# cvigilv/SimSpread.jl

Hardware: AMD Instinct MI355X
Metric: predicted edges/sec + achieved HBM GB/s, W*R SpMM (higher is better)
Workload: dtype f32

## Files before the change

simspread.jl_amd/csrc/kernels.hip:

```cpp
#include <type_traits>

#include "graph.hpp"

namespace ss {

static inline int grid_1d(int64_t work, int block, int cap = 256 * 16) {
  int64_t g = ceil_div(work, block);
  if (g < 1) g = 1;
  if (g > cap) g = cap;
  return (int)g;
}

#define SS_LAUNCH_CHECK()                                                             \
  do {                                                                                \
    hipError_t _e = hipGetLastError();                                                \
    if (_e != hipSuccess)                                                             \
      return fail(SS_EHIP, "%s:%d kernel launch: %s", __FILE__, __LINE__, hipGetErrorString(_e)); \
  } while (0)

template <class T>
__global__ void cutoff_kernel(const T* __restrict__ X, int64_t rows, int64_t cols, int64_t ld, T alpha,
                              int weighted, T* __restrict__ out, int64_t ldo) {
  const int64_t total = rows * cols;
  for (int64_t i = (int64_t)blockIdx.x * blockDim.x + threadIdx.x; i < total;
// ... 853 lines not shown
    const unsigned char* tb = tbl0 + par * W2_TBL;
    int fi, e, qoff;
    bool have = true;
    if (s < 16) {
      fi = 4 * s + (lane >> 4);
      e = lane & 15;
      qoff = 0;
    } else {
      const unsigned char* lst = lst0 + par * 128 + (s < 19 ? 0 : 64);
      const int pos = (s < 19 ? 16 * (s - 16) : 0) + (lane >> 2);
      fi = (int)lst[pos];
      have = fi != 255;
      fi = have ? fi : 0;
      e = lane & 3;
      qoff = s < 19 ? 16 : 20;
    }
    const unsigned* m = reinterpret_cast<const unsigned*>(tb + fi * 12);
    const int b = (int)m[0], n = (int)m[1];
    const float cf = __uint_as_float(m[2]);
    const int qe = qoff + e;
    const bool valid = have && 4 * qe < n;
    fetch(valid ? b + qe : lane, valid ? cf : 0.f, n - 4 * qe, oj, ov, ocf);
  };
  auto fold = [&](u2 j, f4 v, float cf) __attribute__((always_inline)) {
    atomicAdd(acc + (j.x & 0xffffu), (unsigned)cvt_rpi(cf * v.x));
    atomicAdd(acc + (j.x >> 16), (unsigned)cvt_rpi(cf * v.y));
    atomicAdd(acc + (j.y & 0xffffu), (unsigned)cvt_rpi(cf * v.z));
    atomicAdd(acc + (j.y >> 16), (unsigned)cvt_rpi(cf * v.w));
  };
  if (ngroups > 0) {
    raw_load(0, ra, rc);
    open_group(0);
#pragma unroll
    for (int i = 0; i < W2_D; ++i) gen(i, 0, sj[i], sv[i], sc[i]);
    for (int g = 0; g < ngroups; ++g) {
      const int par = g & 1;
#pragma unroll
      for (int s = 0; s < W2_STEPS; ++s) {
        if (s == W2_STEPS - W2_D) open_group(g + 1);
        fold(sj[s % W2_D], sv[s % W2_D], sc[s % W2_D]);
        if (s + W2_D < W2_STEPS) gen(s + W2_D, par, sj[s % W2_D], sv[s % W2_D], sc[s % W2_D]);
        else gen(s + W2_D - W2_STEPS, par ^ 1, sj[s % W2_D], sv[s % W2_D], sc[s % W2_D]);
      }
    }
  }
  float* orow = p.out + r * p.ld + j0;
  const int* iacc = reinterpret_cast<const int*>(acc);
  for (int j = lane; j < jn; j += 64) orow[j] = ((float)iacc[j] * unscale) * p.inv2[j0 + j];
}

template <class T>
static int transfer_block_waves(int64_t mrows, int SC, int* offs_bytes) {
  const int64_t ob = (((mrows + 1) * 4 + 15) / 16) * 16;
  const int64_t per_wave = (int64_t)(SC + 64) * (int64_t)sizeof(T);
  int64_t nw = ((int64_t)ctx().lds_per_block - ob) / per_wave;
  if (ob >= (int64_t)ctx().lds_per_block) nw = 0;
  if (nw > 16) nw = 16;
  if (const char* e = getenv("SS_TRANSFER_NW")) {
    const int v = atoi(e);
    if (v >= 1 && v < nw) nw = v;
  }
  *offs_bytes = (int)ob;
  return nw >= 8 ? (int)nw : 0;
}

template <class T>
int launch_transfer_block(const DevCsr<T>& L, const T* inv1, const DevChunked<T>& Mt, const T* inv2, int64_t row_begin,
                          int64_t nrows, int64_t nj, T* out, int64_t ld, T* coef, float xmax, bool fixed) {
  if (nrows <= 0 || nj <= 0) return SS_OK;
  int offs_bytes = 0;
  const int nw = transfer_block_waves<T>(Mt.rows, Mt.SC, &offs_bytes);
  if (nw == 0) return fail(SS_EUNSUPPORTED, "transfer_block: offsets + accumulators do not fit in LDS");
  TransferArgs<T> p{};
  p.nterms = 1;
  p.L[0] = view(L);
  p.M[0] = view(Mt);
  p.inv2 = inv2;
  p.row_begin = row_begin;
  p.nj = nj;
  p.SC = Mt.SC;
  p.nchunks = Mt.nchunks;
  p.out = out;
  p.ld = ld;
  const int64_t groups = ceil_div(nrows, (int64_t)nw);
  const int64_t grid = groups * p.nchunks;
  if (grid >= (1LL << 31)) return fail(SS_EUNSUPPORTED, "transfer grid too large; lower SS_TRANSFER_BYTES");
  path_add("transfer_block");
  hipLaunchKernelGGL(transfer_coef_kernel<T>, dim3(grid_1d(L.nnz > 0 ? L.nnz : 1, 256, 256 * 8)), dim3(256), 0, ctx().stream,
                     L.ptr.p, L.idx.p, L.val.p, inv1, row_begin, nrows, coef);
  SS_LAUNCH_CHECK();
  const size_t lds = (size_t)offs_bytes + (size_t)nw * (size_t)(p.SC + 64) * sizeof(T);
  constexpr bool CANFIX = std::is_same<T, float>::value;
  const bool fx = CANFIX && fixed;
  if (fx) path_add("fixed_point");
  if constexpr (std::is_same<T, float>::value) {
    auto envi = [](const char* k) { const char* e = getenv(k); return e ? atoi(e) : 0; };
    const int wide2 = envi("SS_TRANSFER_WIDE2"), wide = envi("SS_TRANSFER_WIDE"), qflat = envi("SS_TRANSFER_QFLAT");
    if ((wide2 > 0 || wide > 0 || qflat > 0) && fixed && Mt.align == 32 && Mt.len_ok) {
      const int64_t lens_bytes = ((Mt.rows * 2 + 15) / 16) * 16;
      const int64_t accb = ((((int64_t)p.SC + 4) * 4 + 15) / 16) * 16;
      const int64_t per_wave = wide2 > 0 ? accb + 2 * W2_TBL + 4 * 64
                               : wide > 0 ? accb + WIDE_META + WIDE_LIST : (int64_t)(p.SC + 64) * 4;
      const int64_t fixed_bytes = (int64_t)offs_bytes + lens_bytes + (wide > 0 && wide2 == 0 ? 64 : 0);
      int64_t nwf = ((int64_t)ctx().lds_per_block - fixed_bytes) / per_wave;
      if (nwf > 16) nwf = 16;
      if (const int v = envi("SS_TRANSFER_NW"); v >= 1 && v < nwf) nwf = v;
      if (nwf >= 8) {
        const int64_t fgrid = ceil_div(nrows, nwf) * p.nchunks;
        const size_t flds = (size_t)fixed_bytes + (size_t)nwf * (size_t)per_wave;
        const unsigned short* glen = Mt.len.p;
#define SS_TX_LAUNCH(KERNEL)                                                                                          \
  do {                                                                                                                \
    static std::atomic<bool> attr_done{false};                                                                        \
    if (!attr_done) {                                                                                                 \
      SS_HIP(hipFuncSetAttribute(reinterpret_cast<const void*>(&KERNEL), hipFuncAttributeMaxDynamicSharedMemorySize,  \
                                 160 * 1024));                                                                        \
      attr_done = true;                                                                                               \
    }                                                                                                                 \
    hipLaunchKernelGGL(KERNEL, dim3((unsigned)fgrid), dim3(64 * (int)nwf), flds, ctx().stream, p, (const float*)coef,  \
                       nrows, Mt.align, offs_bytes, (int)lens_bytes, xmax, glen);                                     \
  } while (0)
        if (wide2 > 0) {
          path_add("wide2");
          if (Mt.binary) SS_TX_LAUNCH((transfer_wide2_kernel<true>)); else SS_TX_LAUNCH((transfer_wide2_kernel<false>));
        } else if (wide > 0) {
          path_add("wide");
          if (wide == 2) { if (Mt.binary) SS_TX_LAUNCH((transfer_wide_kernel<2, true>)); else SS_TX_LAUNCH((transfer_wide_kernel<2, false>)); }
          else { if (Mt.binary) SS_TX_LAUNCH((transfer_wide_kernel<4, true>)); else SS_TX_LAUNCH((transfer_wide_kernel<4, false>)); }
        } else {
          path_add("qflat");
          if (Mt.binary) SS_TX_LAUNCH((transfer_qflat_kernel<float, 4, true>)); else SS_TX_LAUNCH((transfer_qflat_kernel<float, 4, false>));
        }
#undef SS_TX_LAUNCH
        SS_LAUNCH_CHECK();
        return SS_OK;
      }
    }
  }
  const int pu = transfer_u() == 4 ? 4 : 8;
#define SS_TB_LAUNCH(U, BINM, FIX)                                                                                    \
  do {                                                                                                                \
    static std::atomic<bool> attr_done{false};                                                                        \
    if (!attr_done) {                                                                                                 \
      SS_HIP(hipFuncSetAttribute(reinterpret_cast<const void*>(&transfer_block_kernel<T, U, BINM, FIX>),              \
                                 hipFuncAttributeMaxDynamicSharedMemorySize, 160 * 1024));                            \
      attr_done = true;                                                                                               \
    }                                                                                                                 \
    hipLaunchKernelGGL((transfer_block_kernel<T, U, BINM, FIX>), dim3((unsigned)grid), dim3(64 * nw), lds,            \
                       ctx().stream, p, (const T*)coef, nrows, Mt.align, offs_bytes, xmax);                           \
  } while (0)
#define SS_TB_BIN(U, FIX) do { if (Mt.binary) SS_TB_LAUNCH(U, true, FIX); else SS_TB_LAUNCH(U, false, FIX); } while (0)
#define SS_TB_FIX(U) do { if (fx) SS_TB_BIN(U, CANFIX); else SS_TB_BIN(U, false); } while (0)
  if (pu == 4) SS_TB_FIX(4);
  else SS_TB_FIX(8);
#undef SS_TB_FIX
#undef SS_TB_BIN
#undef SS_TB_LAUNCH
  SS_LAUNCH_CHECK();
  return SS_OK;
}

template <class T>
bool transfer_block_fits(int64_t mrows, int SC) {
  int ob = 0;
  return transfer_block_waves<T>(mrows, SC, &ob) > 0;
}

template <class T, bool LOO>
static int launch_transfer_variant(const TransferArgs<T>& p, unsigned grid, size_t lds, bool binm, bool dual) {
#define SS_TRANSFER_LAUNCH(U, BINM, DUAL)                                                               \
  hipLaunchKernelGGL((transfer_kernel<T, LOO, U, BINM, DUAL>), dim3(grid), dim3(TRANSFER_THREADS), lds, \
                     ctx().stream, p)
#define SS_TRANSFER_U(U)                                                                      \
  do {                                                                                        \
    if (binm) { if (dual) SS_TRANSFER_LAUNCH(U, true, true); else SS_TRANSFER_LAUNCH(U, true, false); } \
    else { if (dual) SS_TRANSFER_LAUNCH(U, false, true); else SS_TRANSFER_LAUNCH(U, false, false); }    \
  } while (0)
  if constexpr (std::is_same<T, float>::value && !LOO) {
    const char* eb = getenv("SS_TRANSFER_LD");
    if (eb && atoi(eb) == 1 && !dual) {
      path_add("buffer_loads");
      const bool fx = getenv("SS_TRANSFER_FIX1") && atoi(getenv("SS_TRANSFER_FIX1")) == 1 && p.nterms == 1 && !p.accumulate;
      if (fx) path_add("fixed_point");
#define SS_TL(U, BINM, FX) hipLaunchKernelGGL((transfer_kernel<T, LOO, U, BINM, false, FX, true>), dim3(grid), dim3(TRANSFER_THREADS), lds, ctx().stream, p)
      if (transfer_u(p.small_weighted != 0 && !LOO) == 4) {
        if (binm) { if (fx) SS_TL(4, true, true); else SS_TL(4, true, false); }
        else { if (fx) SS_TL(4, false, true); else SS_TL(4, false, false); }
      } else {
        if (binm) { if (fx) SS_TL(8, true, true); else SS_TL(8, true, false); }
        else { if (fx) SS_TL(8, false, true); else SS_TL(8, false, false); }
      }
#undef SS_TL
      SS_LAUNCH_CHECK();
      return SS_OK;
    }
    const char* e = getenv("SS_TRANSFER_FIX1");
    if (e && atoi(e) == 1 && p.nterms == 1 && !dual && !p.accumulate) {
      path_add("fixed_point");
      if (transfer_u(p.small_weighted != 0 && !LOO) == 4) {
        if (binm) hipLaunchKernelGGL((transfer_kernel<T, LOO, 4, true, false, true>), dim3(grid), dim3(TRANSFER_THREADS), lds, ctx().stream, p);
        else hipLaunchKernelGGL((transfer_kernel<T, LOO, 4, false, false, true>), dim3(grid), dim3(TRANSFER_THREADS), lds, ctx().stream, p);
      } else {
        if (binm) hipLaunchKernelGGL((transfer_kernel<T, LOO, 8, true, false, true>), dim3(grid), dim3(TRANSFER_THREADS), lds, ctx().stream, p);
        else hipLaunchKernelGGL((transfer_kernel<T, LOO, 8, false, false, true>), dim3(grid), dim3(TRANSFER_THREADS), lds, ctx().stream, p);
      }
      SS_LAUNCH_CHECK();
      return SS_OK;
    }
  }
  switch (transfer_u(p.small_weighted != 0 && !LOO)) {
    case 4: SS_TRANSFER_U(4); break;
    case 16: SS_TRANSFER_U(16); break;
    default: SS_TRANSFER_U(8); break;
  }
#undef SS_TRANSFER_U
#undef SS_TRANSFER_LAUNCH
  SS_LAUNCH_CHECK();
  return SS_OK;
}

template <class T>
int launch_transfer(int nterms, const DevCsr<T>* L[2], const T* inv1[2], const DevChunked<T>* Mt[2],
                    const T* inv2, int64_t row_begin, int64_t nrows, int64_t nj, T* out, int64_t ld,
                    const int* row_ids, bool accumulate) {
  if (nrows <= 0 || nj <= 0) return SS_OK;
  TransferArgs<T> p{};
  p.nterms = nterms;
  for (int t = 0; t < nterms; ++t) {
    p.L[t] = view(*L[t]);
    p.M[t] = view(*Mt[t]);
    p.inv1[t] = inv1[t];
    if (Mt[t]->SC != Mt[0]->SC || Mt[t]->nchunks != Mt[0]->nchunks)
      return fail(SS_EINVAL, "transfer operands were cut with different chunk sizes");
  }
  p.inv2 = inv2;
  p.row_begin = row_begin;
  p.row_ids = row_ids;
  p.nj = nj;
  p.SC = Mt[0]->SC;
  p.nchunks = Mt[0]->nchunks;
  p.out = out;
  p.ld = ld;
  p.accumulate = accumulate ? 1 : 0;
  p.xmax = 1.0f;
  {
    int64_t bytes = 0;
    bool weighted = false;
    for (int t = 0; t < nterms; ++t) {
      bytes += Mt[t]->stored * (int64_t)(2 + sizeof(T));
      weighted = weighted || !Mt[t]->binary;
    }
    p.small_weighted = (weighted && bytes <= (32LL << 20)) ? 1 : 0;
  }
  p.chunk_interleave = (getenv("SS_TRANSFER_ORDER") && atoi(getenv("SS_TRANSFER_ORDER")) == 0) ? 1 : 0;
  const int64_t grid = nrows * p.nchunks;
  if (grid >= (1LL << 31)) return fail(SS_EUNSUPPORTED, "transfer grid too large; lower SS_TRANSFER_BYTES");
  bool binm = true;
  for (int t = 0; t < nterms; ++t) binm = binm && Mt[t]->binary;
  const bool dual = transfer_dual();
  path_add("transfer");
  const size_t lds = (size_t)(p.SC + 64) * sizeof(T) * (dual ? 2 : 1);
  SS_TRY((launch_transfer_variant<T, false>(p, (unsigned)grid, lds, binm, dual)));
  return SS_OK;
}

template <class T>
int launch_transfer_loo(const DevCsr<T>& X, const DevChunked<T>& XT, const int* kf, const int* ks,
                        int64_t i_begin, int64_t nrows, T* out, int64_t ld) {
  if (nrows <= 0) return SS_OK;
  TransferArgs<T> p{};
  p.nterms = 1;
  p.L[0] = view(X);
  p.M[0] = view(XT);
  p.kf = kf;
  p.ks = ks;
  p.row_begin = i_begin;
  p.nj = X.rows;
  p.SC = XT.SC;
  p.nchunks = XT.nchunks;
  p.out = out;
  p.ld = ld;
  p.chunk_interleave = (getenv("SS_TRANSFER_ORDER") && atoi(getenv("SS_TRANSFER_ORDER")) == 0) ? 1 : 0;
  const int64_t grid = nrows * p.nchunks;
  if (grid >= (1LL << 31)) return fail(SS_EUNSUPPORTED, "transfer grid too large; lower SS_TRANSFER_BYTES");
  const bool dual = transfer_dual();
  path_add("transfer_loo");
  const size_t lds = (size_t)(p.SC + 64) * sizeof(T) * (dual ? 2 : 1) + (size_t)((p.SC + 31) / 32) * 4;
  SS_TRY((launch_transfer_variant<T, true>(p, (unsigned)grid, lds, XT.binary, dual)));
  return SS_OK;
}

template <class T, int QT>
struct alignas(sizeof(T) * QT) Vec {
  T v[QT];
};

template <class T>
struct SellArgs {
  const int* off;
  const unsigned short* idx;
  const T* val;
  int nslices, nchunks, KC;
  int64_t K, M, B;
  const T* R;
  int64_t ldr;
  T* F;
  int64_t ldf;
  const int* clean_deg;
  const int* out_rows;
};

constexpr int SELL_THREADS = 1024;
constexpr int SELL_NB = 4;
constexpr int SELL_QT_F32_DEFAULT = 4;
constexpr int SELL_ZERO_ROWS = 16;
constexpr int SELL_STAGE_IT = 5;

template <int H>
__device__ __forceinline__ unsigned half_shl(unsigned x, unsigned sh) {
  unsigned r;
  if (H == 0)
    asm("v_lshlrev_b32_sdwa %0, %1, %2 dst_sel:DWORD dst_unused:UNUSED_PAD src0_sel:DWORD src1_sel:WORD_0"
        : "=v"(r) : "v"(sh), "v"(x));
  else
    asm("v_lshlrev_b32_sdwa %0, %1, %2 dst_sel:DWORD dst_unused:UNUSED_PAD src0_sel:DWORD src1_sel:WORD_1"
        : "=v"(r) : "v"(sh), "v"(x));
  return r;
}

template <class T, int QT, bool BIN>
__global__ void __launch_bounds__(SELL_THREADS) spmm_sell_kernel(SellArgs<T> a) {
  constexpr int RB = (int)sizeof(T) * QT, NP = RB / 16;
  constexpr int STAGE_IT = NP == 2 ? 2 : SELL_STAGE_IT;
  constexpr int NBQ = NP == 2 ? 2 : SELL_NB;
  constexpr unsigned TSH = NP == 2 ? 5 : 4;
  static_assert(RB == 16 || (RB == 32 && sizeof(T) == 4), "tile row must be 16 bytes, or 32 bytes of fp32");
  extern __shared__ __align__(16) unsigned char smem_raw[];
  using V = Vec<T, QT>;
  V* tile = reinterpret_cast<V*>(smem_raw);
  const int tid = threadIdx.x, lane = tid & 63, wave = tid >> 6, nwaves = blockDim.x >> 6;
  const int64_t b0 = (int64_t)blockIdx.x * QT;
  const unsigned pid = NP == 2 ? (unsigned)(lane & 1) : 0u;

  for (int c = 0; c < a.nchunks; ++c) {
    const int64_t k0 = (int64_t)c * a.KC;
    const int kn = (int)((a.K - k0 < a.KC) ? (a.K - k0) : a.KC);
    if (c) __syncthreads();
    for (int kb = 0; kb < a.KC + SELL_ZERO_ROWS; kb += STAGE_IT * SELL_THREADS) {
      T stg[STAGE_IT][QT];
      const int klast = kn > 0 ? kn - 1 : 0;
#pragma unroll
      for (int it = 0; it < STAGE_IT; ++it) {
        const int k = kb + tid + it * SELL_THREADS;
        const int kk = k < kn ? k : klast;
#pragma unroll
        for (int q = 0; q < QT; ++q) {
          const int64_t b = (b0 + q < a.B) ? b0 + q : a.B - 1;
          stg[it][q] = kn > 0 ? a.R[b * a.ldr + k0 + kk] : T(0);
        }
      }
#pragma unroll
      for (int it = 0; it < STAGE_IT; ++it) {
        const int k = kb + tid + it * SELL_THREADS;
        if (k < a.KC + SELL_ZERO_ROWS) {
          V v;
#pragma unroll
          for (int q = 0; q < QT; ++q) v.v[q] = (k < kn && b0 + q < a.B) ? stg[it][q] : T(0);
          tile[k] = v;
        }
      }
    }
    __syncthreads();

    const int* off = a.off + (int64_t)c * a.nslices;
    const bool last = (c == a.nchunks - 1);
    for (int s = wave + nwaves * (int)blockIdx.y; s < a.nslices; s += nwaves * (int)gridDim.y) {
      const int o = __builtin_amdgcn_readfirstlane(off[s]);
      const int oe = __builtin_amdgcn_readfirstlane(off[s + 1]);
      T acc[QT];
#pragma unroll
      for (int q = 0; q < QT; ++q) acc[q] = T(0);
      const int64_t m = (int64_t)s * 64 + lane;
      T fprev[QT];
#pragma unroll
      for (int q = 0; q < QT; ++q) {
        fprev[q] = T(0);
        if (NP == 1 && c && m < a.M && b0 + q < a.B)
          fprev[q] = a.F[(a.out_rows ? (int64_t)a.out_rows[b0 + q] : b0 + q) * a.ldf + m];
      }
      const ushort4* ip = reinterpret_cast<const ushort4*>(a.idx) + (int64_t)o * 64 + lane;
      const Vec<T, 4>* vp = reinterpret_cast<const Vec<T, 4>*>(a.val) + (int64_t)o * 64 + lane;
      const uint2* ipw = reinterpret_cast<const uint2*>(ip);
      const int nq = oe - o;
      uint2 ia[NBQ], ib[NBQ];
      Vec<T, 4> wa[NBQ], wb[NBQ];
      auto fetch = [&](uint2 (&iq)[NBQ], Vec<T, 4> (&wq)[NBQ], int base) __attribute__((always_inline)) {
#pragma unroll
        for (int j = 0; j < NBQ; ++j) {
          iq[j] = ipw[(int64_t)(base + j) * 64];
          if (!BIN) wq[j] = vp[(int64_t)(base + j) * 64];
        }
      };
      auto gather = [&](const uint2 (&iq)[NBQ], const Vec<T, 4> (&wq)[NBQ], int cnt) __attribute__((always_inline)) {
        constexpr int PV = 16 / (int)sizeof(T);
        typedef T NV __attribute__((ext_vector_type(PV)));
        using LV = const __attribute__((address_space(3))) NV*;
        const unsigned lb = pid << 4;
        auto row = [&](unsigned addr) __attribute__((always_inline)) {
          V r;
          if (NP == 1) {
            const NV n = *(LV)(uintptr_t)addr;
#pragma unroll
            for (int q = 0; q < PV; ++q) r.v[q] = n[q];
          } else {
            const unsigned a0 = addr | lb;
            const NV n0 = *(LV)(uintptr_t)a0;
            const NV n1 = *(LV)(uintptr_t)(a0 ^ 16u);
#pragma unroll
            for (int q = 0; q < PV; ++q) { r.v[q] = n0[q]; r.v[PV + q] = n1[q]; }
          }
          return r;
        };
#pragma unroll
        for (int j = 0; j < NBQ; ++j) {
          if (j >= cnt) break;
          const V t0 = row(half_shl<0>(iq[j].x, TSH));
          const V t1 = row(half_shl<1>(iq[j].x, TSH));
          const V t2 = row(half_shl<0>(iq[j].y, TSH));
          const V t3 = row(half_shl<1>(iq[j].y, TSH));
          if (BIN) {
#pragma unroll
            for (int q = 0; q < QT; ++q) acc[q] += (t0.v[q] + t1.v[q]) + (t2.v[q] + t3.v[q]);
          } else {
#pragma unroll
            for (int q = 0; q < QT; ++q) {
              acc[q] = fma(wq[j].v[0], t0.v[q], acc[q]);
              acc[q] = fma(wq[j].v[1], t1.v[q], acc[q]);
              acc[q] = fma(wq[j].v[2], t2.v[q], acc[q]);
              acc[q] = fma(wq[j].v[3], t3.v[q], acc[q]);
            }
          }
          if (NP == 2) __builtin_amdgcn_sched_barrier(0);
        }
      };
      fetch(ia, wa, 0);
      fetch(ib, wb, NBQ);
      int u = 0;
      for (; u + 2 * NBQ <= nq; u += 2 * NBQ) {
        gather(ia, wa, NBQ);
        fetch(ia, wa, u + 2 * NBQ);
        gather(ib, wb, NBQ);
        fetch(ib, wb, u + 3 * NBQ);
      }
      {
        const int rest = nq - u;
        if (rest > 0) gather(ia, wa, rest < NBQ ? rest : NBQ);
        if (rest > NBQ) gather(ib, wb, rest - NBQ);
      }
      if (m < a.M) {
        const bool flag = last && a.clean_deg != nullptr && a.clean_deg[m] == 0;
#pragma unroll
        for (int q = 0; q < QT; ++q) {
          if (b0 + q < a.B) {
            T* f = a.F + (a.out_rows ? (int64_t)a.out_rows[b0 + q] : b0 + q) * a.ldf + m;
            const T mine = NP == 2 ? (pid ? acc[q ^ (QT / 2)] : acc[q]) : acc[q];
            const T r = mine + ((NP == 2 && c) ? *f : fprev[q]);
            *f = flag ? T(-99) : r;
          }
        }
      }
    }
  }
}

template <> int sell_tile_width<float>() {
  if (const char* e = getenv("SS_SELL_QT")) {
    const int v = atoi(e);
    if (v == 4 || v == 8) return v;
  }
  return SELL_QT_F32_DEFAULT;
}
template <> int sell_tile_width<double>() { return 2; }

template <class T>
int sell_max_chunk(int qt) {
  int64_t kc = (int64_t)(160 * 1024) / ((int64_t)qt * (int64_t)sizeof(T)) - SELL_ZERO_ROWS;
  if (kc > 65535 - (SELL_ZERO_ROWS - 1)) kc = 65535 - (SELL_ZERO_ROWS - 1);
  return (int)kc;
}

template <class T>
int launch_spmm_sell(const DevSell<T>& W, const T* R, int64_t ldr, int64_t B, T* F, int64_t ldf,
                     const int* clean_deg, const int* out_rows) {
  if (B <= 0 || W.rows <= 0) return SS_OK;
  path_add(W.sorted ? "spmm_sell_sorted" : "spmm_sell");
  const int QT = W.qt > 0 ? W.qt : (sizeof(T) == 4 ? 4 : 2);
  SellArgs<T> a{};
  a.off = W.off.p;
  a.idx = W.idx.p;
  a.val = W.val.p;
  a.nslices = W.nslices;
  a.nchunks = W.nchunks;
  a.KC = W.KC;
  a.K = W.cols;
  a.M = W.sorted ? W.vrows : W.rows;
  a.B = B;
  a.R = R;
  a.ldr = ldr;
  a.F = F;
  a.ldf = ldf;
  a.clean_deg = clean_deg;
  a.out_rows = out_rows;
  const size_t lds = (size_t)(W.KC + SELL_ZERO_ROWS) * QT * sizeof(T);
  if (lds > (size_t)160 * 1024) return fail(SS_EINVAL, "SELL chunk does not fit the LDS tile of %d columns", QT);
  const unsigned gx = (unsigned)ceil_div(B, QT);
  unsigned gy = 1;
  if ((int)gx < 2 * ctx().num_cu) {
    gy = (unsigned)ceil_div(2 * ctx().num_cu, (int64_t)gx);
    const unsigned maxy = (unsigned)ceil_div(W.nslices, SELL_THREADS / 64);
    if (gy > maxy) gy = maxy > 0 ? maxy : 1;
  }
  const dim3 grid(gx, gy);
  auto prepare = [](const void* fn) -> int {
    hipFuncAttributes fa{};
    SS_HIP(hipFuncGetAttributes(&fa, fn));
    if (fa.sharedSizeBytes != 0)
      return fail(SS_EUNSUPPORTED, "spmm_sell_kernel was built with %zu bytes of static LDS: its tile-relative LDS "
                  "addresses need the dynamic segment at LDS address 0", (size_t)fa.sharedSizeBytes);
    SS_HIP(hipFuncSetAttribute(fn, hipFuncAttributeMaxDynamicSharedMemorySize, 160 * 1024));
    return SS_OK;
  };
#define SS_SELL_LAUNCH(QTV, BINV, SLOT)                                                                      \
  do {                                                                                                       \
    static std::atomic<bool> attr_done{false};                                                               \
    if (!attr_done) {                                                                                        \
      SS_TRY(prepare(reinterpret_cast<const void*>(&spmm_sell_kernel<T, QTV, BINV>)));                       \
      attr_done = true;                                                                                      \
    }                                                                                                        \
    hipLaunchKernelGGL((spmm_sell_kernel<T, QTV, BINV>), grid, dim3(SELL_THREADS), lds, ctx().stream, a);    \
  } while (0)
  if constexpr (sizeof(T) == 4) {
    if (QT == 8) { if (W.binary) SS_SELL_LAUNCH(8, true, 0); else SS_SELL_LAUNCH(8, false, 1); }
    else if (QT == 4) { if (W.binary) SS_SELL_LAUNCH(4, true, 2); else SS_SELL_LAUNCH(4, false, 3); }
    else return fail(SS_EINVAL, "SELL tile width must be 4 or 8 (fp32)");
  } else {
    if (QT != 2) return fail(SS_EINVAL, "SELL tile width must be 2 (fp64)");
    if (W.binary) SS_SELL_LAUNCH(2, true, 0); else SS_SELL_LAUNCH(2, false, 1);
  }
#undef SS_SELL_LAUNCH
  SS_LAUNCH_CHECK();
  return SS_OK;
}

template <class T>
struct NarrowArgs {
  const int* off;
  const unsigned short* idx;
  const T* val;
  int64_t M, K;
  int KC, nchunks, B;
  const T* R;
  int64_t ldr;
  T* F;
  int64_t ldf;
  T* P;
};

constexpr int NARROW_THREADS = 1024;

template <int CTRL, int ROW_MASK = 0xF>
__device__ __forceinline__ float dpp_add(float v) {
  return v + __int_as_float(__builtin_amdgcn_update_dpp(0, __float_as_int(v), CTRL, ROW_MASK, 0xF, false));
}
template <int CTRL, int ROW_MASK = 0xF>
__device__ __forceinline__ double dpp_add(double v) {
  const long long b = __double_as_longlong(v);
  const int lo = __builtin_amdgcn_update_dpp(0, (int)(b & 0xffffffffll), CTRL, ROW_MASK, 0xF, false);
  const int hi = __builtin_amdgcn_update_dpp(0, (int)(b >> 32), CTRL, ROW_MASK, 0xF, false);
  return v + __longlong_as_double(((long long)hi << 32) | (unsigned int)lo);
}
template <int GL, class T>
__device__ __forceinline__ T lane_group_sum(T v) {
  static_assert(GL == 8 || GL == 16 || GL == 32 || GL == 64, "group of 8, 16, 32 or 64 lanes");
  v = dpp_add<0xB1>(v);
  v = dpp_add<0x4E>(v);
  v = dpp_add<0x141>(v);
  if constexpr (GL >= 16) v = dpp_add<0x140>(v);
  if constexpr (GL >= 32) v = dpp_add<0x142, 0xA>(v);
  if constexpr (GL >= 64) v = dpp_add<0x143, 0xC>(v);
  return v;
}

template <class T, int VEC, int GL, int UR, int NBQ>
__global__ void __launch_bounds__(NARROW_THREADS) spmm_chunked_narrow_kernel(NarrowArgs<T> a) {
  constexpr int BV = VEC;
  extern __shared__ __align__(16) unsigned char smem_raw[];
  T* tile = reinterpret_cast<T*>(smem_raw);
  using V = Vec<T, VEC>;
  const int tid = threadIdx.x, lane = tid & 63, wave = tid >> 6, nwaves = blockDim.x >> 6;
  const int c = blockIdx.x % a.nchunks;
  const int slot = blockIdx.x / a.nchunks, nslots = gridDim.x / a.nchunks;
  const int64_t k0 = (int64_t)c * a.KC;
  const int kn = (int)((a.K - k0 < a.KC) ? (a.K - k0) : a.KC);

  constexpr bool SWZ = (BV * sizeof(T) == 32);
  constexpr int HB = 16 / (int)sizeof(T);
  constexpr int PW16 = 16 / (int)sizeof(T);
  const bool packed = a.ldr == BV && a.B == BV &&
                      ((reinterpret_cast<uintptr_t>(a.R + k0 * a.ldr) & 15) == 0) && ((a.KC * BV) % PW16 == 0);
  if (packed) {
    using P16 = Vec<T, PW16>;
    const P16* __restrict__ src = reinterpret_cast<const P16*>(a.R + k0 * a.ldr);
    P16* dst = reinterpret_cast<P16*>(tile);
    const int npieces = ((a.KC + 1) * BV + PW16 - 1) / PW16, nfull = (kn * BV) / PW16;
    for (int i = tid; i < npieces; i += blockDim.x) {
      P16 v;
      if (i < nfull) {
        v = src[i];
      } else {
#pragma unroll
        for (int e = 0; e < PW16; ++e) {
          const int x = i * PW16 + e;
          v.v[e] = (x < kn * BV) ? a.R[k0 * a.ldr + x] : T(0);
        }
      }
      if ((i + 1) * PW16 <= (a.KC + 1) * BV) {
        dst[SWZ ? (i ^ ((i >> 4) & 1)) : i] = v;
      } else {
#pragma unroll
        for (int e = 0; e < PW16; ++e)
          if (i * PW16 + e < (a.KC + 1) * BV) tile[i * PW16 + e] = v.v[e];
      }
    }
  } else {
    for (int e = tid; e < (a.KC + 1) * BV; e += blockDim.x) {
      const int k = e / BV, b = e - k * BV;
      const T v = (k < kn && b < a.B) ? a.R[(k0 + k) * a.ldr + b] : T(0);
      if constexpr (SWZ) tile[k * BV + ((((b / HB) ^ (k >> 3)) & 1) * HB) + (b % HB)] = v;
      else tile[e] = v;
    }
  }
  __syncthreads();
  auto tile_row = [&](int k) __attribute__((always_inline)) {
    V r;
    if constexpr (SWZ) {
      using H = Vec<T, HB>;
      const int s = (k >> 3) & 1;
      const H lo = *reinterpret_cast<const H*>(&tile[k * BV + s * HB]);
      const H hi = *reinterpret_cast<const H*>(&tile[k * BV + (s ^ 1) * HB]);
#pragma unroll
      for (int i = 0; i < HB; ++i) { r.v[i] = lo.v[i]; r.v[HB + i] = hi.v[i]; }
    } else {
      r = *reinterpret_cast<const V*>(&tile[k * BV]);
    }
    return r;
  };

  const int* __restrict__ off = a.off + (int64_t)c * a.M;
  {
    constexpr int RPS = 64 / GL;
    const int sub = lane / GL, gl = lane % GL;
    const ushort4* __restrict__ ip = reinterpret_cast<const ushort4*>(a.idx);
    const Vec<T, 4>* __restrict__ vp = reinterpret_cast<const Vec<T, 4>*>(a.val);
    const int64_t stride = (int64_t)nslots * nwaves * RPS * UR;
    struct Bounds { int lo[UR], hi[UR]; };
    struct Quads { ushort4 iv[UR][NBQ]; Vec<T, 4> w[UR][NBQ]; unsigned mask; };
    auto bounds = [&](int64_t mb, Bounds& b) __attribute__((always_inline)) {
#pragma unroll
      for (int u = 0; u < UR; ++u) {
        const int64_t m = mb + u * RPS + sub;
        const int64_t mm = m < a.M ? m : a.M - 1;
        b.lo[u] = off[mm];
        b.hi[u] = off[mm + 1];
      }
    };
    auto issue = [&](int64_t mb, const Bounds& b, Quads& x) __attribute__((always_inline)) {
      unsigned mask = 0;
#pragma unroll
      for (int u = 0; u < UR; ++u) {
        const int oe = (mb + u * RPS + sub < a.M) ? b.hi[u] : b.lo[u];
#pragma unroll
        for (int nb = 0; nb < NBQ; ++nb) {
          const int q = b.lo[u] + gl + nb * GL;
          const bool in = q < oe;
          const int qq = in ? q : b.lo[u];
          {
            typedef unsigned nt_u2 __attribute__((ext_vector_type(2)));
            typedef T nt_t4 __attribute__((ext_vector_type(4)));
            const nt_u2 ii = __builtin_nontemporal_load(reinterpret_cast<const nt_u2*>(&ip[qq]));
            const nt_t4 ww = __builtin_nontemporal_load(reinterpret_cast<const nt_t4*>(&vp[qq]));
            x.iv[u][nb] = ushort4((unsigned short)(ii.x & 0xffffu), (unsigned short)(ii.x >> 16), (unsigned short)(ii.y & 0xffffu),
                                  (unsigned short)(ii.y >> 16));
            x.w[u][nb].v[0] = ww.x; x.w[u][nb].v[1] = ww.y; x.w[u][nb].v[2] = ww.z; x.w[u][nb].v[3] = ww.w;
          }
          mask |= in ? (1u << (u * NBQ + nb)) : 0u;
        }
        mask |= (b.lo[u] + NBQ * GL < oe) ? 0x80000000u : 0u;
      }
      x.mask = mask;
    };
    auto quad = [&](T (&acc)[VEC], const ushort4 jv, const Vec<T, 4> x) __attribute__((always_inline)) {
      const V r0 = tile_row((int)jv.x);
      const V r1 = tile_row((int)jv.y);
      const V r2 = tile_row((int)jv.z);
      const V r3 = tile_row((int)jv.w);
#pragma unroll
      for (int i = 0; i < VEC; ++i) {
        acc[i] = fma(x.v[0], r0.v[i], acc[i]);
        acc[i] = fma(x.v[1], r1.v[i], acc[i]);
        acc[i] = fma(x.v[2], r2.v[i], acc[i]);
        acc[i] = fma(x.v[3], r3.v[i], acc[i]);
      }
    };
    int64_t mb = ((int64_t)slot * nwaves + wave) * RPS * UR;
    Bounds bn;
    Quads xa, xb;
    if (mb < a.M) {
      Bounds b0;
      bounds(mb, b0);
      bounds(mb + stride < a.M ? mb + stride : mb, bn);
      issue(mb, b0, xa);
    }
    auto step = [&](const int64_t mb, const Quads& xc, Quads& xn) __attribute__((always_inline)) {
      const int64_t mb1 = mb + stride < a.M ? mb + stride : mb;
      const int64_t mb2 = mb + 2 * stride < a.M ? mb + 2 * stride : mb;
      Bounds bnn;
      bounds(mb2, bnn);
      issue(mb1, bn, xn);
      __builtin_amdgcn_sched_barrier(0);
      T acc[UR][VEC];
#pragma unroll
      for (int u = 0; u < UR; ++u) {
#pragma unroll
        for (int i = 0; i < VEC; ++i) acc[u][i] = T(0);
#pragma unroll
        for (int nb = 0; nb < NBQ; ++nb) {
          const bool has = (xc.mask >> (u * NBQ + nb)) & 1u;
          Vec<T, 4> w = xc.w[u][nb];
#pragma unroll
          for (int e = 0; e < 4; ++e) w.v[e] = has ? w.v[e] : T(0);
          quad(acc[u], xc.iv[u][nb], w);
        }
      }
      if (__any((int)(xc.mask >> 31))) {
#pragma unroll
        for (int u = 0; u < UR; ++u) {
          const int64_t m = mb + u * RPS + sub;
          if (m < a.M) {
            const int lo = off[m], hi = off[m + 1];
            for (int q = lo + gl + NBQ * GL; q < hi; q += GL) quad(acc[u], ip[q], vp[q]);
          }
        }
      }
#pragma unroll
      for (int u = 0; u < UR; ++u) {
#pragma unroll
        for (int i = 0; i < VEC; ++i) acc[u][i] = lane_group_sum<GL>(acc[u][i]);
        const int64_t m = mb + u * RPS + sub;
        if (gl == GL - 1 && m < a.M) {
          if (a.P) {
            T* p = a.P + ((int64_t)c * a.M + m) * BV;
#pragma unroll
            for (int i = 0; i < VEC; ++i) p[i] = acc[u][i];
          } else {
#pragma unroll
            for (int i = 0; i < VEC; ++i)
              if (i < a.B) a.F[m * a.ldf + i] = acc[u][i];
          }
        }
      }
      bn = bnn;
    };
    while (mb < a.M) {
      step(mb, xa, xb);
      mb += stride;
      if (mb >= a.M) break;
      step(mb, xb, xa);
      mb += stride;
    }
  }
}

template <class T, int BV>
__global__ void narrow_reduce_kernel(const T* __restrict__ P, int nchunks, int64_t M, int B, T* __restrict__ F,
                                     int64_t ldf) {
  using PV = Vec<T, BV>;
  for (int64_t m = (int64_t)blockIdx.x * blockDim.x + threadIdx.x; m < M; m += (int64_t)gridDim.x * blockDim.x) {
    PV s = *reinterpret_cast<const PV*>(P + m * BV);
    for (int c = 1; c < nchunks; ++c) {
      const PV t = *reinterpret_cast<const PV*>(P + ((int64_t)c * M + m) * BV);
#pragma unroll
      for (int e = 0; e < BV; ++e) s.v[e] += t.v[e];
    }
#pragma unroll
    for (int e = 0; e < BV; ++e)
      if (e < B) F[m * ldf + e] = s.v[e];
  }
}

template <class T>
int narrow_chunk_cols(int bv) {
  int64_t kc = (int64_t)(160 * 1024) / ((int64_t)bv * (int64_t)sizeof(T)) - 1;
  if (kc > 65535) kc = 65535;
  kc &= ~3LL;
  return (int)kc;
}

template <class T, int VEC, int GL, int UR, int NBQ = 1>
static int launch_narrow_variant(const NarrowArgs<T>& a, unsigned grid, size_t lds) {
  static std::atomic<bool> attr_set{false};
  if (!attr_set) {
    SS_HIP(hipFuncSetAttribute(reinterpret_cast<const void*>(&spmm_chunked_narrow_kernel<T, VEC, GL, UR, NBQ>),
                               hipFuncAttributeMaxDynamicSharedMemorySize, 160 * 1024));
    attr_set = true;
  }
  hipLaunchKernelGGL((spmm_chunked_narrow_kernel<T, VEC, GL, UR, NBQ>), dim3(grid), dim3(NARROW_THREADS), lds,
                     ctx().stream, a);
  SS_LAUNCH_CHECK();
  return SS_OK;
}

constexpr int narrow_ur(int elem, int vec, int nbq) {
  const int per_quad = 2 + elem;
  int ur = 4;
  while (ur > 1 && 2 * ur * nbq * per_quad + (ur + 4) * vec * (elem / 4) + 4 * ur + 24 > 124) ur >>= 1;
  return ur;
}

template <class T, int VEC>
static int launch_narrow_width(const NarrowArgs<T>& a, unsigned grid, size_t lds, double mean_quads) {
  constexpr int E = (int)sizeof(T);
  const double need = 1.1 * mean_quads + 1.0;
  if (need > 64.0) return launch_narrow_variant<T, VEC, 64, narrow_ur(E, VEC, 2), 2>(a, grid, lds);
  if (need > 32.0) return launch_narrow_variant<T, VEC, 64, narrow_ur(E, VEC, 1)>(a, grid, lds);
  if (need > 16.0) return launch_narrow_variant<T, VEC, 32, narrow_ur(E, VEC, 1)>(a, grid, lds);
  if (need > 8.0) return launch_narrow_variant<T, VEC, 16, narrow_ur(E, VEC, 1)>(a, grid, lds);
  return launch_narrow_variant<T, VEC, 8, narrow_ur(E, VEC, 1)>(a, grid, lds);
}

template <class T>
int launch_spmm_chunked_narrow(const DevChunked<T>& W, int bv, const T* R, int64_t ldr, int B, T* F, int64_t ldf,
                               DevBuf<T>& partial) {
  if (W.rows <= 0 || B <= 0) return SS_OK;
  if (W.align != 4) return fail(SS_EINVAL, "narrow operand must be quad-aligned");
  path_add("spmm_chunked_narrow");
  NarrowArgs<T> a{};
  a.off = W.off.p; a.idx = W.idx.p; a.val = W.val.p;
  a.M = W.rows; a.K = W.cols; a.KC = W.SC; a.nchunks = W.nchunks; a.B = B;
  a.R = R; a.ldr = ldr; a.F = F; a.ldf = ldf; a.P = nullptr;
  if (W.nchunks > 1) {
// ... 440 lines not shown
```

Baseline: 48.95 billion.

## Make SELL SpMM persistent and prefetch next tile's R staging during compute

The SELL SpMM kernel becomes persistent when gy==1: the grid is capped at the CU count and each workgroup loops over column tiles and chunks. Global loads of R for the first two staging rounds of the next tile or chunk are issued into registers before the following sync, so they overlap the current compute. This targets the exposed latency of filling the LDS tile and the cost of launching many short workgroups. In exchange it raises register pressure and launches fewer workgroups. It also adds env knobs, including a NOSTAGE debug variant.

```diff
diff --git a/simspread.jl_amd/csrc/kernels.hip b/simspread.jl_amd/csrc/kernels.hip
--- a/simspread.jl_amd/csrc/kernels.hip
+++ b/simspread.jl_amd/csrc/kernels.hip
@@ -1179,6 +1179,7 @@
   const T* val;
   int nslices, nchunks, KC;
   int64_t K, M, B;
+  int64_t ntiles;
   const T* R;
   int64_t ldr;
   T* F;
@@ -1205,10 +1206,11 @@
   return r;
 }
 
-template <class T, int QT, bool BIN>
+template <class T, int QT, bool BIN, bool NOSTAGE = false>
 __global__ void __launch_bounds__(SELL_THREADS) spmm_sell_kernel(SellArgs<T> a) {
   constexpr int RB = (int)sizeof(T) * QT, NP = RB / 16;
   constexpr int STAGE_IT = NP == 2 ? 2 : SELL_STAGE_IT;
+  constexpr int RND = STAGE_IT * SELL_THREADS;
   constexpr int NBQ = NP == 2 ? 2 : SELL_NB;
   constexpr unsigned TSH = NP == 2 ? 5 : 4;
   static_assert(RB == 16 || (RB == 32 && sizeof(T) == 4), "tile row must be 16 bytes, or 32 bytes of fp32");
@@ -1216,36 +1218,53 @@
   using V = Vec<T, QT>;
   V* tile = reinterpret_cast<V*>(smem_raw);
   const int tid = threadIdx.x, lane = tid & 63, wave = tid >> 6, nwaves = blockDim.x >> 6;
-  const int64_t b0 = (int64_t)blockIdx.x * QT;
   const unsigned pid = NP == 2 ? (unsigned)(lane & 1) : 0u;
 
-  for (int c = 0; c < a.nchunks; ++c) {
+  const int trows = a.KC + SELL_ZERO_ROWS;
+  auto request = [&](T (&stg)[STAGE_IT][QT], int64_t b0, int c, int kb) __attribute__((always_inline)) {
     const int64_t k0 = (int64_t)c * a.KC;
     const int kn = (int)((a.K - k0 < a.KC) ? (a.K - k0) : a.KC);
-    if (c) __syncthreads();
-    for (int kb = 0; kb < a.KC + SELL_ZERO_ROWS; kb += STAGE_IT * SELL_THREADS) {
-      T stg[STAGE_IT][QT];
-      const int klast = kn > 0 ? kn - 1 : 0;
-#pragma unroll
-      for (int it = 0; it < STAGE_IT; ++it) {
-        const int k = kb + tid + it * SELL_THREADS;
-        const int kk = k < kn ? k : klast;
-#pragma unroll
-        for (int q = 0; q < QT; ++q) {
-          const int64_t b = (b0 + q < a.B) ? b0 + q : a.B - 1;
-          stg[it][q] = kn > 0 ? a.R[b * a.ldr + k0 + kk] : T(0);
-        }
-      }
-#pragma unroll
-      for (int it = 0; it < STAGE_IT; ++it) {
-        const int k = kb + tid + it * SELL_THREADS;
-        if (k < a.KC + SELL_ZERO_ROWS) {
-          V v;
-#pragma unroll
-          for (int q = 0; q < QT; ++q) v.v[q] = (k < kn && b0 + q < a.B) ? stg[it][q] : T(0);
-          tile[k] = v;
-        }
-      }
+    const int klast = kn > 0 ? kn - 1 : 0;
+    const T* rq[QT];
+#pragma unroll
+    for (int q = 0; q < QT; ++q) rq[q] = a.R + ((b0 + q < a.B) ? b0 + q : a.B - 1) * a.ldr + k0;
+#pragma unroll
+    for (int it = 0; it < STAGE_IT; ++it) {
+      const int k = kb + tid + it * SELL_THREADS;
+      const unsigned kk = (unsigned)(k < kn ? k : klast);
+#pragma unroll
+      for (int q = 0; q < QT; ++q) stg[it][q] = NOSTAGE ? T(1) : rq[q][kk];
+    }
+  };
+  auto deposit = [&](const T (&stg)[STAGE_IT][QT], int64_t b0, int kn, int kb) __attribute__((always_inline)) {
+#pragma unroll
+    for (int it = 0; it < STAGE_IT; ++it) {
+      const int k = kb + tid + it * SELL_THREADS;
+      if (k < trows) {
+        V v;
+#pragma unroll
+        for (int q = 0; q < QT; ++q) v.v[q] = (k < kn && b0 + q < a.B) ? stg[it][q] : T(0);
+        tile[k] = v;
+      }
+    }
+  };
+
+  int64_t t = blockIdx.x;
+  if (t >= a.ntiles) return;
+  int c = 0;
+  T sta[STAGE_IT][QT], stb[STAGE_IT][QT];
+  request(sta, t * QT, c, 0);
+  request(stb, t * QT, c, RND);
+  for (;;) {
+    const int64_t b0 = t * QT;
+    const int64_t k0 = (int64_t)c * a.KC;
+    const int kn = (int)((a.K - k0 < a.KC) ? (a.K - k0) : a.KC);
+    deposit(sta, b0, kn, 0);
+    deposit(stb, b0, kn, RND);
+    for (int kb = 2 * RND; kb < trows; kb += RND) {
+      T stc[STAGE_IT][QT];
+      request(stc, b0, c, kb);
+      deposit(stc, b0, kn, kb);
     }
     __syncthreads();
 
@@ -1347,6 +1366,21 @@
         }
       }
     }
+    int cn = c + 1;
+    int64_t tn = t;
+    if (cn == a.nchunks) {
+      cn = 0;
+      tn = t + gridDim.x;
+    }
+    const bool more = tn < a.ntiles;
+    if (more) {
+      t = tn;
+      c = cn;
+    }
+    request(sta, t * QT, c, 0);
+    request(stb, t * QT, c, RND);
+    if (!more) break;
+    __syncthreads();
   }
 }
 
@@ -1388,15 +1422,25 @@
   a.ldf = ldf;
   a.clean_deg = clean_deg;
   a.out_rows = out_rows;
+  if (W.cols == 0) {
+    a.R = reinterpret_cast<const T*>(W.off.p);
+    a.ldr = 0;
+  }
   const size_t lds = (size_t)(W.KC + SELL_ZERO_ROWS) * QT * sizeof(T);
   if (lds > (size_t)160 * 1024) return fail(SS_EINVAL, "SELL chunk does not fit the LDS tile of %d columns", QT);
-  const unsigned gx = (unsigned)ceil_div(B, QT);
+  const unsigned ntiles = (unsigned)ceil_div(B, QT);
+  a.ntiles = ntiles;
   unsigned gy = 1;
-  if ((int)gx < 2 * ctx().num_cu) {
-    gy = (unsigned)ceil_div(2 * ctx().num_cu, (int64_t)gx);
+  if ((int)ntiles < 2 * ctx().num_cu) {
+    gy = (unsigned)ceil_div(2 * ctx().num_cu, (int64_t)ntiles);
     const unsigned maxy = (unsigned)ceil_div(W.nslices, SELL_THREADS / 64);
     if (gy > maxy) gy = maxy > 0 ? maxy : 1;
   }
+  auto envi = [](const char* k, int dflt) { const char* e = getenv(k); return e ? atoi(e) : dflt; };
+  unsigned gx = ntiles;
+  if (gy == 1 && envi("SS_SELL_PERSIST", 1) != 0 && (unsigned)ctx().num_cu < gx) gx = (unsigned)ctx().num_cu;
+  if (const int cap = envi("SS_SELL_WGS", 0); cap > 0 && (unsigned)cap < gx) gx = (unsigned)cap;
+  const bool nostage = envi("SS_SELL_NOSTAGE", 0) == 1;
   const dim3 grid(gx, gy);
   auto prepare = [](const void* fn) -> int {
     hipFuncAttributes fa{};
@@ -1407,22 +1451,24 @@
     SS_HIP(hipFuncSetAttribute(fn, hipFuncAttributeMaxDynamicSharedMemorySize, 160 * 1024));
     return SS_OK;
   };
-#define SS_SELL_LAUNCH(QTV, BINV, SLOT)                                                                      \
+#define SS_SELL_LAUNCH(QTV, BINV, ...)                                                                       \
   do {                                                                                                       \
     static std::atomic<bool> attr_done{false};                                                               \
     if (!attr_done) {                                                                                        \
-      SS_TRY(prepare(reinterpret_cast<const void*>(&spmm_sell_kernel<T, QTV, BINV>)));                       \
+      SS_TRY(prepare(reinterpret_cast<const void*>(&spmm_sell_kernel<T, QTV, BINV, ##__VA_ARGS__>)));        \
       attr_done = true;                                                                                      \
     }                                                                                                        \
-    hipLaunchKernelGGL((spmm_sell_kernel<T, QTV, BINV>), grid, dim3(SELL_THREADS), lds, ctx().stream, a);    \
+    hipLaunchKernelGGL((spmm_sell_kernel<T, QTV, BINV, ##__VA_ARGS__>), grid, dim3(SELL_THREADS), lds,       \
+                       ctx().stream, a);                                                                     \
   } while (0)
   if constexpr (sizeof(T) == 4) {
-    if (QT == 8) { if (W.binary) SS_SELL_LAUNCH(8, true, 0); else SS_SELL_LAUNCH(8, false, 1); }
-    else if (QT == 4) { if (W.binary) SS_SELL_LAUNCH(4, true, 2); else SS_SELL_LAUNCH(4, false, 3); }
+    if (QT == 8) { if (W.binary) SS_SELL_LAUNCH(8, true); else SS_SELL_LAUNCH(8, false); }
+    else if (QT == 4 && nostage) { if (W.binary) SS_SELL_LAUNCH(4, true, true); else SS_SELL_LAUNCH(4, false, true); }
+    else if (QT == 4) { if (W.binary) SS_SELL_LAUNCH(4, true); else SS_SELL_LAUNCH(4, false); }
     else return fail(SS_EINVAL, "SELL tile width must be 4 or 8 (fp32)");
   } else {
     if (QT != 2) return fail(SS_EINVAL, "SELL tile width must be 2 (fp64)");
-    if (W.binary) SS_SELL_LAUNCH(2, true, 0); else SS_SELL_LAUNCH(2, false, 1);
+    if (W.binary) SS_SELL_LAUNCH(2, true); else SS_SELL_LAUNCH(2, false);
   }
 #undef SS_SELL_LAUNCH
   SS_LAUNCH_CHECK();
```

Result: no change. 49.01 billion, median of 4 (+0.1%).
